# ruanyyyyyyy/point-cloud-process

Hardware: AMD Instinct MI355X
Metric: correspondence-pairs/sec + ms/ICP-iter, 120k-pt KITTI pair (higher is better)
Workload: dtype f64; 1 GPU; point-to-point ICP iteration, 120000 x 120000 KITTI-shaped synthetic scan pair per GPU (BASELINE configs[1]); exact 1-NN via grid; nn=grid, pairs_per_gpu=1, points_src=120000, points_tgt=120000

## Files before the change

include/pcr.h:

```cpp
#ifndef PCR_H
#define PCR_H

#include <stdint.h>

#ifdef __cplusplus
extern "C" {
#endif

#define PCR_API __attribute__((visibility("default")))

enum {
    PCR_OK = 0,
    PCR_E_TOO_FEW_ASSOC = 1,
    PCR_E_INVALID = -1,
    PCR_E_EMPTY = -2,
    PCR_E_NOMEM = -3,
    PCR_E_HIP = -4,
    PCR_E_NO_DEVICE = -5,
    PCR_E_UNSUPPORTED = -6,
    PCR_E_TOO_MANY_ITERS = -7,
    PCR_E_SINGULAR = -8
};

typedef struct pcr_ctx pcr_ctx;
// ... 257 lines not shown
    int32_t reserved_i;
    double inertia;
    double shift;
    double device_ms;
    double reserved[4];
} pcr_kmeans_result;
PCR_API void pcr_kmeans_default_params(pcr_kmeans_params* p);
PCR_API int pcr_kmeans_fit(pcr_ctx* ctx, const pcr_cloud* cloud, const pcr_kmeans_params* params, const double* centers0 ,
                           double* centers_out , int64_t* counts_out , int32_t* labels_out, double* inertia_hist_out,
                           double* shift_hist_out, pcr_kmeans_result* result);
PCR_API int pcr_kmeans_step(pcr_ctx* ctx, const pcr_cloud* cloud, int k, int dim, const double* centers, double* centers_out, int64_t* counts_out,
                            double* sums_out, double* inertia_out, double* shift_out);
PCR_API int pcr_kmeans_predict(pcr_ctx* ctx, const pcr_cloud* cloud, int k, int dim, const double* centers, int32_t* labels_out, int64_t* counts_out,
                               double* inertia_out);
PCR_API int pcr_cloud_download_rows(pcr_ctx* ctx, const pcr_cloud* cloud, const int64_t* rows , int64_t m, double* xyz_out );

PCR_API int pcr_timer_start(pcr_ctx* ctx);
PCR_API int pcr_timer_stop_ms(pcr_ctx* ctx, double* ms_out);
PCR_API int pcr_debug_read(pcr_ctx* ctx, uint64_t* out, int64_t n_words);
PCR_API int pcr_profile_enable(pcr_ctx* ctx, int on);
PCR_API int pcr_search_stats(pcr_ctx* ctx, int64_t out[4]);

PCR_API int pcr_icp_pass_log(pcr_ctx* ctx, int max_n, double* tile_us, double* drain_us, int64_t* items, int* n_out, double host_us[6]);

PCR_API int pcr_ctx_set_shared(pcr_ctx* ctx, int shared);
PCR_API int pcr_profile_read(pcr_ctx* ctx, double ms_out[4], int* passes_out);

#ifdef __cplusplus
}
#endif
#endif
```

point-cloud-process_amd/_lib.py:

```python
from __future__ import annotations

import ctypes as C
import os
import sys

import numpy as np

_HERE = os.path.dirname(os.path.abspath(__file__))
LIB_PATH = os.environ.get("PCR_LIB_PATH") or os.path.join(_HERE, "libpcr.so")

PCR_OK = 0
PCR_E_TOO_FEW_ASSOC = 1
PCR_E_INVALID = -1
PCR_E_EMPTY = -2
PCR_E_NOMEM = -3
PCR_E_HIP = -4
PCR_E_NO_DEVICE = -5
PCR_E_UNSUPPORTED = -6
PCR_E_TOO_MANY_ITERS = -7
PCR_E_SINGULAR = -8

PCR_INDEX_GRID = 0
PCR_INDEX_BRUTE = 1
PCR_ICP_COMPAT_MAIN = 0
# ... 253 lines not shown
    "pcr_prep_download": (C.c_int, [_vp, _vp, _dp, _dp, _dp]),
    "pcr_prep_free": (C.c_int, [_vp, _vp]),
    "pcr_global_registration": (C.c_int, [_vp, _vp, _vp, C.POINTER(RansacParams), C.c_int, C.POINTER(RansacResult)]),
    "pcr_dbscan": (C.c_int, [_vp, _vp, C.c_double, C.c_int, _ip, _ip]),
    "pcr_ground_default_params": (None, [C.POINTER(GroundParams)]),
    "pcr_ground_select": (C.c_int, [_lp, C.c_int32, C.c_int64, C.c_double, _ip, _ip]),
    "pcr_ground_segmentation": (C.c_int, [_vp, _vp, _lp, C.POINTER(GroundParams), C.POINTER(_vp), _ip, C.POINTER(C.c_uint8), _lp, C.POINTER(GroundResult)]),
    "pcr_gmm_default_params": (None, [C.POINTER(GmmParams)]),
    "pcr_gmm_fit": (C.c_int, [_vp, _vp, C.POINTER(GmmParams), _dp, _dp, _dp, _dp, _dp, C.POINTER(GmmResult)]),
    "pcr_gmm_step": (C.c_int, [_vp, _vp, C.c_int, C.c_int, _dp, _dp, _dp, _dp, _dp, _dp, _dp, _dp]),
    "pcr_gmm_predict": (C.c_int, [_vp, _vp, C.c_int, C.c_int, _dp, _dp, _dp, _ip, _dp, _dp]),
    "pcr_gmm_log_density": (C.c_int, [C.c_int, _dp, _dp, _dp, C.c_double, _dp]),
    "pcr_kmeans_default_params": (None, [C.POINTER(KmeansParams)]),
    "pcr_kmeans_fit": (C.c_int, [_vp, _vp, C.POINTER(KmeansParams), _dp, _dp, _lp, _ip, _dp, _dp, C.POINTER(KmeansResult)]),
    "pcr_kmeans_step": (C.c_int, [_vp, _vp, C.c_int, C.c_int, _dp, _dp, _lp, _dp, _dp, _dp]),
    "pcr_kmeans_predict": (C.c_int, [_vp, _vp, C.c_int, C.c_int, _dp, _ip, _lp, _dp]),
    "pcr_cloud_download_rows": (C.c_int, [_vp, _vp, _lp, C.c_int64, _dp]),
    "pcr_debug_read": (C.c_int, [_vp, C.POINTER(C.c_uint64), C.c_int64]),
    "pcr_profile_enable": (C.c_int, [_vp, C.c_int]),
    "pcr_profile_read": (C.c_int, [_vp, _dp, C.POINTER(C.c_int)]),
    "pcr_search_stats": (C.c_int, [_vp, _lp]),
    "pcr_ctx_set_shared": (C.c_int, [_vp, C.c_int]),
    "pcr_icp_pass_log": (C.c_int, [_vp, C.c_int, _dp, _dp, _lp, C.POINTER(C.c_int), _dp]),
    "pcr_timer_start": (C.c_int, [_vp]),
    "pcr_timer_stop_ms": (C.c_int, [_vp, _dp]),
}

_lib = None


class PcrError(RuntimeError):
    def __init__(self, status, detail=""):
        self.status = status
        msg = f"libpcr status {status}"
        try:
            msg += ": " + lib().pcr_strerror(status).decode()
        except Exception:
            pass
        if detail:
            msg += f" ({detail})"
        super().__init__(msg)


def lib():
    global _lib
    if _lib is not None:
# ... 47 lines not shown
```

point-cloud-process_amd/csrc/pcr_core.hip:

```cpp
#include <cmath>
#include <cstdio>
#include <cstring>
#include <cstdlib>
#include <chrono>
#include <thread>
#include <atomic>
#include <memory>
#include "pcr_internal.h"

extern "C" {

const char* pcr_version(void) { return "pcr 0.1 (gfx950, f64)"; }

const char* pcr_strerror(int s) {
    switch (s) {
        case PCR_OK: return "ok";
        case PCR_E_TOO_FEW_ASSOC: return "ICP failed, cannot find enough associations!";
        case PCR_E_INVALID: return "invalid argument";
        case PCR_E_EMPTY: return "empty point cloud";
        case PCR_E_NOMEM: return "out of memory";
        case PCR_E_HIP: return "HIP runtime error";
        case PCR_E_NO_DEVICE: return "no HIP device (libpcr.so needs an AMD GPU; there is no CPU fallback)";
        case PCR_E_UNSUPPORTED: return "unsupported";
        case PCR_E_TOO_MANY_ITERS: return "max_iter exceeds PCR_ICP_MAX_LOG";
// ... 248 lines not shown
    if (!c || !out) return PCR_E_INVALID;
    hipSetDevice(c->device);
    unsigned int fb = 0;
    int rc = pcr_brute_last_fallback(c, &fb);
    if (rc) return rc;
    out[0] = fb;
    out[1] = c->arena_grow_count;
    out[2] = (int64_t)c->arena_grow_us;
    out[3] = (int64_t)c->arenas.size();
    return PCR_OK;
}

int pcr_icp_pass_log(pcr_ctx* c, int max_n, double* tile_us, double* drain_us, int64_t* items, int* n_out, double host_us[6]) {
    if (!c || !n_out || max_n < 0) return PCR_E_INVALID;
    const int n = c->pass_log_n < max_n ? c->pass_log_n : max_n;
    for (int k = 0; k < n; ++k) {
        if (tile_us) tile_us[k] = c->pass_log[0][k];
        if (drain_us) drain_us[k] = c->pass_log[1][k];
        if (items) items[k] = (int64_t)c->pass_log[2][k];
    }
    *n_out = c->pass_log_n;
    if (host_us)
        for (int k = 0; k < 6; ++k) host_us[k] = c->pass_host_us[k];
    return PCR_OK;
}

int pcr_timer_start(pcr_ctx* c) {
    if (!c) return PCR_E_INVALID;
    PCR_HIP(c, hipEventRecord(c->ev2, c->stream));
    return PCR_OK;
}

int pcr_timer_stop_ms(pcr_ctx* c, double* ms) {
    if (!c || !ms) return PCR_E_INVALID;
    PCR_HIP(c, hipEventRecord(c->ev3, c->stream));
    PCR_HIP(c, pcr_event_sync(c->ev3));
    float f = 0;
    PCR_HIP(c, hipEventElapsedTime(&f, c->ev2, c->ev3));
    *ms = f;
    return PCR_OK;
}

}

void pcr_prof_mark(pcr_ctx* ctx, int k) {
    if (ctx->profile) hipEventRecord(ctx->pev[k], ctx->stream);
// ... 324 lines not shown
```

point-cloud-process_amd/csrc/pcr_grid_search.hip:

```cpp
#include <atomic>
#include <chrono>
#include <cmath>
#include <cstdlib>
#include <cstring>
#include "pcr_descent.h"
#include "pcr_icp_step.h"

constexpr unsigned int HARD_SCAN_T = 192;
constexpr int HARD_STACK = 160;
constexpr long long ID_NONE = 0x7fffffffffffffffll;
constexpr int H_NLIST = 32;
constexpr int H_CSTRIDE = 32;
__host__ __device__ static inline unsigned int hard_list_cap(long long nq) {
    const long long halves = (nq + 15) / 16;
    return (unsigned int)(((halves + H_NLIST - 1) / H_NLIST) * 16 + 64);
}

template <int G>
__device__ static inline void group_best(double& bd2, long long& bid, unsigned int& bpos) {
#pragma unroll
    for (int off = G / 2; off > 0; off >>= 1) {
        const double od2 = __shfl_xor(bd2, off, 64);
        const long long oid = __shfl_xor(bid, off, 64);
        const unsigned int opos = __shfl_xor(bpos, off, 64);
// ... 461 lines not shown
    S.won = won;
    S.open = open; S.clamped = clamped; S.qvalid = qvalid;
    S.staged = staged;
    S.dbg_pairs = dbg_pairs; S.dbg_passes = dbg_passes;
    {
        const bool ok = lane < (int)probe_groups && (unsigned int)probe_v == probe_total / (probe_groups ? probe_groups : 1u) + ((unsigned int)lane < probe_total % (probe_groups ? probe_groups : 1u) ? 1u : 0u);
        S.probe = (probe_groups && __ballot(ok) == (probe_groups >= 64 ? ~0ull : (1ull << probe_groups) - 1ull)) ? 1ull : 0ull;
    }
#ifdef PCR_WT_DIAG
    if (dbg) {
        const bool unres = open && lane < WT_Q;
        for (int r = 0; r < 5; ++r) {
            const unsigned int n_r = (unsigned int)__popcll(__ballot(unres && (clamped ? 0 : why) == r));
            if (lane == 0 && n_r) atomicAdd(&dbg[(1 << 15) + r], (unsigned long long)n_r);
        }
        if (lane == 0) {
            t_ph[7] = staged;
            for (int i = 0; i < 8; ++i) dbg[(1 << 16) + (blockIdx.x * 4 + (threadIdx.x >> 6)) * 8 + i] = t_ph[i];
        }
    }
#endif
}

__device__ static inline unsigned int wtile_block(int xcd_remap) {
    unsigned int blk = blockIdx.x;
    if (xcd_remap) {
        const unsigned int per = gridDim.x >> 3, main = per << 3;
        if (blk < main) blk = (blk & 7u) * per + (blk >> 3);
    }
    return blk;
}

__global__ void __launch_bounds__(256) __attribute__((amdgpu_waves_per_eu(PCR_WT_WAVES, 8)))
grid_wtile_kernel(const pcr_grid_view* __restrict__ gvp, pcr_pt* __restrict__ q, long long nq, pcr_xform x, int has_x, int write_back, double max_d2,
                  int gated, int xcd_remap, unsigned int pcap, unsigned int* __restrict__ res_pos, double* __restrict__ res_d2,
                  work_item* __restrict__ hard_list, unsigned int* __restrict__ hard_count, unsigned long long* __restrict__ dbg,
                  const pcr_icp_dev_state* __restrict__ st, const wt_xyz* __restrict__ prev_xyz) {
    __shared__ wtile_lds s_lds[4];
    if (st) {
        if (st->stop) return;
        x = st->x;
    }
    const unsigned long long t_start = dbg ? __builtin_amdgcn_s_memtime() : 0;
    const int lane = threadIdx.x & 63, wave = threadIdx.x >> 6;
    const unsigned int blk = wtile_block(xcd_remap);
    wt_state S;
    wt_pre P;
    wtile_preload(blk * 4 + wave, lane, q, nq, res_pos, prev_xyz, P);
    wtile_search(*gvp, &s_lds[wave], blk * 4 + wave, lane, P, q, nq, x, has_x, write_back, max_d2, gated, pcap, res_pos, res_d2, dbg, prev_xyz, S);
    const bool unres = S.open && lane < WT_Q;
// ... 276 lines not shown
constexpr unsigned long long ITEM_NONE = ~0ull;
constexpr unsigned int POISON_HI = 0xfffffffeu;
__device__ static inline unsigned long long item_poison(unsigned int pass_id) { return ((unsigned long long)POISON_HI << 32) | pass_id; }
#ifndef PCR_PASS_SPIN_LIMIT
#define PCR_PASS_SPIN_LIMIT (1u << 21)
#endif
constexpr unsigned int PASS_SPIN_LIMIT = PCR_PASS_SPIN_LIMIT;
constexpr int Q_BITS = 22;
constexpr unsigned long long Q_MASK = (1ull << Q_BITS) - 1ull;
constexpr long long PASS_MAX_NQ = 1ll << 26;
struct pass_args {
    unsigned long long* items;
    unsigned long long* sync;
    unsigned int cap;
    unsigned long long* acc;
    wt_xyz* prev_xyz;
    double scale, inv_scale;
    pcr_icp_dev_state* st;
    pcr_icp_loop_args la;
    unsigned int* tile_cost;
    unsigned int pass_id;
    unsigned long long* host_block;
    unsigned int notify;
    unsigned int* plog;
};
constexpr int PASS_LOG_WORDS = 3 * PCR_ICP_MAX_LOG + 8;
constexpr size_t HOST_LOG_OFF = (sizeof(pcr_icp_dev_state) + 63) & ~(size_t)63;
constexpr size_t HOST_FLAG_OFF = 8192 - 8;
static_assert(HOST_LOG_OFF + 4 * PASS_LOG_WORDS <= HOST_FLAG_OFF, "state + pass log + flag fit the landing block");
__host__ __device__ static inline unsigned int pass_item_cap(long long nq) {
    const long long tiles = (nq + WT_Q - 1) / WT_Q + 4;
    return (unsigned int)(((tiles + PASS_GROUPS - 1) / PASS_GROUPS) * (WT_Q + 1));
}

__device__ static inline long long to_fixed(double v, double scale) {
    constexpr double BIG = 6755399441055744.0;
    return __double_as_longlong(__builtin_fma(v, scale, BIG)) - __double_as_longlong(BIG);
}

__device__ static inline void acc_fixed_add(unsigned long long* __restrict__ acc, unsigned int set, int lane, double mk, double scale) {
    if (lane < PCR_NMOM - 1 && mk != 0.0)
        atomicAdd(acc + (size_t)(set % ACC_SETS) * PCR_NMOM + lane, (unsigned long long)to_fixed(mk, scale));
}

__device__ static inline void acc_fixed_add_ll(unsigned long long* __restrict__ acc, unsigned int set, int lane, long long v) {
    if (lane < PCR_NMOM - 1 && v != 0) atomicAdd(acc + (size_t)(set % ACC_SETS) * PCR_NMOM + lane, (unsigned long long)v);
}

__device__ static inline unsigned long long ld_dev(const unsigned long long* p) {
    return __hip_atomic_load(p, __ATOMIC_RELAXED, __HIP_MEMORY_SCOPE_AGENT);
}
__device__ static inline void st_dev(unsigned long long* p, unsigned long long v) {
    __hip_atomic_store(p, v, __ATOMIC_RELAXED, __HIP_MEMORY_SCOPE_AGENT);
}

union pass_lds {
    wtile_lds t;
    hard_lds h;
    double xch[WT_Q * (PCR_NMOM - 1)];
    long long xll[WT_Q * (PCR_NMOM - 1)];
};

__device__ __forceinline__ static void pass_serve_item(const pcr_grid_view& gv, pass_lds* L, const int lane, const unsigned long long w, const double max_d2,
                                                       const pass_args& A, unsigned int* __restrict__ res_pos, unsigned long long* __restrict__ dbg,
                                                       const unsigned int dbg_slot, const unsigned long long t_start) {
    const unsigned int w_lo = (unsigned int)w, w_hi = (unsigned int)(w >> 32);
    const double ax = __hiloint2double(__builtin_amdgcn_readlane((int)w_hi, 0), __builtin_amdgcn_readlane((int)w_lo, 0));
    const double ay = __hiloint2double(__builtin_amdgcn_readlane((int)w_hi, 1), __builtin_amdgcn_readlane((int)w_lo, 1));
    const double az = __hiloint2double(__builtin_amdgcn_readlane((int)w_hi, 2), __builtin_amdgcn_readlane((int)w_lo, 2));
    const unsigned int qi = (unsigned int)__builtin_amdgcn_readlane((int)w_lo, 3);
    const float cand_b2 = __uint_as_float((unsigned int)__builtin_amdgcn_readlane((int)w_hi, 3));
    const unsigned long long h_t0 = dbg ? __builtin_amdgcn_s_memtime() : 0;
    unsigned int h_steps = 0, h_pts = 0;
    int s_level0 = 0;
    double bd2;
    long long bid;
    unsigned int bpos;
    const bool have_cand = cand_b2 < INFINITY;
    double win[3];
    hard_search(gv, &L->h, lane, ax, ay, az, have_cand ? fmin((double)cand_b2, max_d2) : max_d2, have_cand, bd2, bid, bpos, h_steps, h_pts, s_level0, win);
    wave_sync();
    if (bpos != POS_NONE) {
        if (lane == 0) {
// ... 155 lines not shown

struct drain_part {
    unsigned int cnt, exc, total;
};
__device__ __forceinline__ static drain_part drain_partition(const unsigned long long* sync, int lane) {
    static_assert(PASS_GROUPS <= 64, "one group per lane");
    drain_part d;
    d.cnt = lane < PASS_GROUPS ? (unsigned int)(sync[(size_t)PASS_SYNC_STRIDE * lane] & Q_MASK) : 0u;
    d.exc = wave_excl_scan_u32(d.cnt, lane, &d.total);
    return d;
}
__device__ __forceinline__ static unsigned long long drain_take(const drain_part& d, unsigned long long* items, unsigned int cap, unsigned int w_i, int lane) {
    const int grp = (int)__ffsll((long long)__ballot(((lane < PASS_GROUPS) & (d.exc <= w_i)) && w_i < d.exc + d.cnt)) - 1;
    const unsigned int idx = w_i - (unsigned int)__builtin_amdgcn_readlane((int)d.exc, grp);
    unsigned long long* it = items + ((size_t)grp * cap + idx) * 4;
    unsigned long long w = ITEM_NONE;
    if (lane < 4) {
        w = it[lane];
        it[lane] = ITEM_NONE;
    }
    return w;
}

#ifndef PCR_PASS_DIAG
#define PCR_PASS_DIAG 0
#endif
__global__ void __launch_bounds__(256) __attribute__((amdgpu_waves_per_eu(PCR_WT_WAVES, 8)))
grid_pass_kernel(const pcr_grid_view* __restrict__ gvp, pcr_grid_view gv, pcr_pt* __restrict__ q, long long nq, double max_d2, int xcd_remap,
                 unsigned int pcap_arg, unsigned int pcap_busy, unsigned int* __restrict__ res_pos, unsigned long long* __restrict__ dbg_arg, int use_prev, int inline_queue,
                 pass_args A) {
    unsigned long long* const dbg = PCR_PASS_DIAG ? dbg_arg : nullptr;
    __shared__ pass_lds s_lds[4];
    const int lane = threadIdx.x & 63, wave = __builtin_amdgcn_readfirstlane((int)(threadIdx.x >> 6));
    const unsigned int tile = wtile_block(xcd_remap) * 4 + wave;
    wt_pre P;
    wtile_preload(tile, lane, q, nq, res_pos, use_prev ? A.prev_xyz : nullptr, P);
    const unsigned int last_cost = use_prev ? A.tile_cost[tile] : 0u;
    unsigned int pcap = pcap_arg;
    if (pcap_busy > pcap_arg && A.plog) {
        const unsigned int prev_items = A.pass_id > 0 && A.pass_id <= (unsigned int)PCR_ICP_MAX_LOG ? A.plog[2 * PCR_ICP_MAX_LOG + A.pass_id - 1] : 0xffffffffu;
        if ((unsigned long long)prev_items * 16ull > (unsigned long long)nq) pcap = pcap_busy;
        pcap = (unsigned int)__builtin_amdgcn_readfirstlane((int)pcap);
    }
    const pcr_xform x = A.st->x;
    if (A.st->stop) return;
    tile_set_priority(last_cost);
    const unsigned long long t_start = dbg ? __builtin_amdgcn_s_memtime() : 0;
    const unsigned long long rt_start = dbg ? __builtin_amdgcn_s_memrealtime() : 0;
    unsigned long long rt_tile = 0, rt_acc = 0;
    unsigned int n_items = 0, n_polls = 0, n_casfail = 0;
    pass_lds* L = &s_lds[wave];
    const unsigned int n_waves = gridDim.x * 4;
    const unsigned int g = tile % PASS_GROUPS;
    const unsigned int g_tiles = n_waves / PASS_GROUPS + (g < n_waves % PASS_GROUPS ? 1u : 0u);
    unsigned long long* const g_q = A.sync + (size_t)PASS_SYNC_STRIDE * g;
    unsigned long long* const g_started = g_q + 16;
    unsigned long long* const g_ticket = g_q + 17;
    unsigned long long* const items = A.items + (size_t)g * A.cap * 4;
    if (lane == 0) __hip_atomic_fetch_add(g_started, 1ull, __ATOMIC_RELAXED, __HIP_MEMORY_SCOPE_AGENT);
    const unsigned int n_groups = n_waves < (unsigned int)PASS_GROUPS ? n_waves : (unsigned int)PASS_GROUPS;
    wt_state S;
    wtile_search(*gvp, &L->t, tile, lane, P, q, nq, x, 1, 1, max_d2, 1, pcap, res_pos, nullptr, dbg, use_prev ? A.prev_xyz : nullptr, S, inline_queue ? A.sync + 16 : nullptr,
                 (unsigned int)PASS_SYNC_STRIDE, n_groups, n_waves);
    tile_record_cost(S, lane, A.tile_cost, tile);
    if (dbg) rt_tile = __builtin_amdgcn_s_memrealtime();
    tile_nb nb;
    tile_neighbour(gv.pts, S, P, lane, nb);
    bool all_started = false;
    if (inline_queue) {
        all_started = S.probe != 0;
        if (!all_started) {
            unsigned long long sv = 0;
            if (lane < (int)n_groups) sv = ld_dev(A.sync + (size_t)PASS_SYNC_STRIDE * lane + 16);
            const bool ok = lane < (int)n_groups && (unsigned int)sv == n_waves / PASS_GROUPS + ((unsigned int)lane < n_waves % PASS_GROUPS ? 1u : 0u);
            all_started = __ballot(ok) == (n_groups >= 64 ? ~0ull : (1ull << n_groups) - 1ull);
// ... 100 lines not shown
        pass_serve_item(gv, L, lane, w, max_d2, A, res_pos, dbg, g + PASS_GROUPS * mine, t_start);
    }
    const unsigned long long rt_loop = dbg ? __builtin_amdgcn_s_memrealtime() : 0;
    asm volatile("s_waitcnt vmcnt(0)" ::: "memory");
    int last = 0;
    {
        if (lane == 0) {
            const unsigned long long tg_old = __hip_atomic_fetch_add(g_ticket, 1ull | (left_by_poison ? 1ull << 32 : 0ull) | (failed ? 1ull << 48 : 0ull), __ATOMIC_RELAXED,
                                                                     __HIP_MEMORY_SCOPE_AGENT);
            if ((unsigned int)tg_old == g_tiles - 1u) {
                const bool g_clean = ((tg_old >> 32) & 0xffffull) != 0 || left_by_poison;
                const bool g_failed = (tg_old >> 48) != 0 || failed;
                const unsigned long long tr_old = __hip_atomic_fetch_add(root, 1ull | (g_clean ? 1ull << 32 : 0ull) | (g_failed ? 1ull << 48 : 0ull), __ATOMIC_RELAXED,
                                                                         __HIP_MEMORY_SCOPE_AGENT);
                if ((unsigned int)tr_old == n_groups - 1u) {
                    last = ((unsigned int)((tr_old >> 32) & 0xffffull) + (g_clean ? 1u : 0u) == n_groups) ? 1 : 2;
                    if ((tr_old >> 48) != 0 || g_failed) last = 3;
                }
            }
        }
    }
    if (dbg && lane == 0) {
        unsigned long long* d = dbg + (1 << 19) + (size_t)(blockIdx.x * 4 + wave) * 8;
        d[0] = rt_start; d[1] = rt_tile; d[2] = rt_acc; d[3] = rt_loop; d[4] = n_items; d[5] = n_polls | ((unsigned long long)n_casfail << 32); d[6] = S.dbg_pairs | ((unsigned long long)S.dbg_passes << 40) | ((unsigned long long)__popcll(um) << 48); d[7] = __builtin_amdgcn_s_memrealtime();
    }
    last = __builtin_amdgcn_readfirstlane(last);
    if (!last) return;
    if (last == 3 && dbg_arg && lane == 0) atomicAdd(&dbg_arg[(1 << 19) - 16], 1ull);
    if (last >= 2) {
        unsigned long long qw = 0;
        if (lane < (int)n_groups) qw = ld_dev(A.sync + (size_t)PASS_SYNC_STRIDE * lane);
        const unsigned int r_l = (unsigned int)(qw & Q_MASK);
        const unsigned int c_l = last == 3 ? 0u : (unsigned int)((qw >> Q_BITS) & Q_MASK);
        unsigned long long left = __ballot(lane < (int)n_groups && c_l < r_l);
        while (left) {
            const int gg = (int)__ffsll((long long)left) - 1;
            left &= left - 1;
            const unsigned int c0 = (unsigned int)__builtin_amdgcn_readlane((int)c_l, gg), r0 = (unsigned int)__builtin_amdgcn_readlane((int)r_l, gg);
            for (unsigned int i = c0; i < r0; ++i) {
                unsigned long long* it = A.items + ((size_t)gg * A.cap + i) * 4;
                unsigned long long w = ITEM_NONE;
                bool arrived = false;
                const unsigned int patience = last == 3 ? 64u : (PASS_SPIN_LIMIT < (1u << 21) ? (1u << 21) : PASS_SPIN_LIMIT);
                bool served_before = false;
                for (unsigned int spins = 0; spins < patience; ++spins) {
                    if (lane < 4) w = ld_dev(it + lane);
                    const unsigned int w3_hi = (unsigned int)__builtin_amdgcn_readlane((int)(unsigned int)(w >> 32), 3);
// ... 188 lines not shown
        __syncthreads();
        if (threadIdx.x == 0) pcr::icp_step(st, s_m, gv.origin, la, st->r_diff, st->t_diff);
    }
}

struct grid_scratch {
    pcr_dev_block res_pos, res_d2;
    pcr_dev_block hard_list;
    pcr_dev_block prev_xyz;
    pcr_dev_block acc, items, tile_cost;
    unsigned int* const hard_count;
    explicit grid_scratch(pcr_ctx* ctx)
        : res_pos(ctx), res_d2(ctx), hard_list(ctx), prev_xyz(ctx), acc(ctx), items(ctx), tile_cost(ctx), hard_count(ctx->d_counters + PCR_HARD_COUNTERS) {}
};

static int grid_scratch_alloc(grid_scratch* sc, int64_t nq, bool want_d2, bool want_hard) {
    int rc;
    if ((rc = sc->res_pos.alloc(sizeof(unsigned int) * nq))) return rc;
    if (want_d2 && (rc = sc->res_d2.alloc(sizeof(double) * nq))) return rc;
    if (want_hard && (rc = sc->hard_list.alloc(sizeof(work_item) * (size_t)H_NLIST * hard_list_cap(nq)))) return rc;
    return PCR_OK;
}

struct pass_layout {
    size_t sync_word, log_word, zero_words;
    unsigned int cap;
    unsigned long long item_words;
};
static pass_layout pass_scratch_layout(long long nq, int n_pairs, bool with_log) {
    pass_layout l;
    l.sync_word = (size_t)n_pairs * ACC_SETS * PCR_NMOM;
    l.log_word = l.sync_word + PASS_SYNC_WORDS;
    l.zero_words = l.log_word + (with_log ? PASS_LOG_WORDS / 2 : 0);
    l.cap = pass_item_cap(nq);
    l.item_words = 4ull * PASS_GROUPS * l.cap;
    return l;
}

static int wtile_blocks(int64_t nq) { return (int)((nq + 4 * WT_Q - 1) / (4 * WT_Q)); }
static int queue_blocks(const pcr_ctx* ctx, long long want) { return (int)(want < 8ll * ctx->cu_count ? (want < 1 ? 1 : want) : 8ll * ctx->cu_count); }

static unsigned int wtile_point_cap(const pcr_ctx* ctx, int64_t nq) {
    const int nblocks = (int)((nq + 63) / 64);
    return (unsigned int)WT_PR * (nblocks > 8 * ctx->cu_count ? WT_ROUNDS_LARGE : WT_ROUNDS_SMALL);
}
constexpr unsigned int WT_BUSY_CAP = WT_PR * 48;
constexpr int WT_XCD_REMAP = 1;

static int grid_search_enqueue(pcr_ctx* ctx, const pcr_index* idx, pcr_pt* q, int64_t nq, hipStream_t stream, const pcr_xform* x, int write_back,
                               double max_d2, bool gated, bool mark, const grid_scratch* sc, const pcr_icp_dev_state* st, bool use_prev = false) {
    const int nblocks = (int)((nq + 63) / 64);
    pcr_xform xi;
    pcr_xform_from_T(nullptr, &xi);
    if (mark) pcr_prof_mark(ctx, 0);
    {
        if (ctx->d_debug) hipMemsetAsync(ctx->d_debug, 0, sizeof(unsigned long long) * ((1 << 16) + 8 * (size_t)nblocks), stream);
        hipLaunchKernelGGL(grid_wtile_kernel, dim3(wtile_blocks(nq)), dim3(256), 0, stream, (const pcr_grid_view*)idx->d_view, q, (long long)nq, x ? *x : xi,
                           (x || st) ? 1 : 0, write_back, max_d2, gated ? 1 : 0, WT_XCD_REMAP, wtile_point_cap(ctx, nq), sc->res_pos.as<unsigned int>(),
                           sc->res_d2.as<double>(), sc->hard_list.as<work_item>(), sc->hard_count, ctx->d_debug, st, (const wt_xyz*)(use_prev ? sc->prev_xyz.p : nullptr));
    }
    if (mark) pcr_prof_mark(ctx, 1);
    hipLaunchKernelGGL(grid_hard_kernel, dim3(queue_blocks(ctx, (nq + 3) / 4)), dim3(256), 0, stream, idx->view, (const work_item*)sc->hard_list.p,
// ... 77 lines not shown
    frexp(M / (double)nq, &exq);
    const int F = (61 - ex < 51 - exq) ? 61 - ex : 51 - exq;
    if (!(M > 0) || !std::isfinite(M) || F < 20) return false;
    *scale = ldexp(1.0, F);
    *inv_scale = ldexp(1.0, -F);
    return true;
}

static std::atomic<int> g_loops_in_flight[64];
struct loop_guard {
    std::atomic<int>& n;
    explicit loop_guard(int device) : n(g_loops_in_flight[(unsigned int)device % 64u]) { n.fetch_add(1); }
    ~loop_guard() { n.fetch_sub(1); }
};

int pcr_grid_icp_loop(pcr_ctx* ctx, const pcr_index* idx, pcr_cloud* qc, const pcr_icp_params* params, const double T0[16],
                      pcr_icp_result* res) {
    const loop_guard in_flight(ctx->device);
    const auto h_t0 = std::chrono::steady_clock::now();
    auto h_us = [&](std::chrono::steady_clock::time_point a) { return std::chrono::duration_cast<std::chrono::nanoseconds>(std::chrono::steady_clock::now() - a).count() / 1e3; };
    for (double& v : ctx->pass_host_us) v = 0.0;
    const char* const wait_s = getenv("PCR_PASS_INLINE");
    const int wait_env = wait_s ? atoi(wait_s) : -1;
    const bool gated = (params->max_d2 > 0) && std::isfinite(params->max_d2);
    int rc = pcr_cloud_morton_sort(ctx, qc, idx->cell);
    if (rc) return rc;
    const int64_t nq = qc->n;
    int grid = (int)((nq + 1023) / 1024);
    if (grid > ctx->cu_count) grid = ctx->cu_count;
    double sc_f = 0, sc_i = 0;
    const bool fused = gated && nq <= PASS_MAX_NQ && getenv("PCR_ICP_NO_FUSED") == nullptr &&
                       pcr_pass_fixed_scale(idx->lo, idx->hi, nq, params->max_d2, &sc_f, &sc_i);
    grid_scratch sc(ctx);
    pcr_dev_block st_blk(ctx);
    if ((rc = grid_scratch_alloc(&sc, nq, false, !fused)) || (rc = sc.prev_xyz.alloc(24 * (size_t)nq))) return rc;
    const pass_layout pl = pass_scratch_layout(nq, 1, true);
    pass_args pa{};
    if (fused) {
        if ((rc = sc.acc.alloc(8 * pl.zero_words)) || (rc = sc.tile_cost.alloc(sizeof(unsigned int) * 4 * (size_t)wtile_blocks(nq))) ||
            (rc = sc.items.alloc(8 * pl.item_words)))
            return rc;
        pa.cap = pl.cap;
        pa.items = sc.items.as<unsigned long long>();
        pa.tile_cost = sc.tile_cost.as<unsigned int>();
        pa.acc = sc.acc.as<unsigned long long>();
        pa.sync = pa.acc + pl.sync_word;
        pa.plog = (unsigned int*)(pa.acc + pl.log_word);
        pa.prev_xyz = sc.prev_xyz.as<wt_xyz>();
        pa.scale = sc_f;
        pa.inv_scale = sc_i;
    }
    if ((rc = pcr_ensure_scratch(ctx, sizeof(double) * PCR_NMOM * (size_t)grid)) || (rc = st_blk.alloc(sizeof(pcr_icp_dev_state)))) return rc;
    pcr_icp_dev_state* const d_st = st_blk.as<pcr_icp_dev_state>();
    static_assert(sizeof(pcr_icp_dev_state) <= 8192, "state must fit the pinned staging buffer");
    pcr_icp_dev_state* h_st = (pcr_icp_dev_state*)ctx->h_state;
    memset(h_st, 0, sizeof(*h_st));
    pcr::icp_state_from_T0(T0, h_st);
    const pcr_icp_loop_args la = pcr_icp_loop_args_from(params);
    volatile unsigned long long* const h_flag = (volatile unsigned long long*)((char*)ctx->h_state + HOST_FLAG_OFF);
    if (fused) {
        void* dp = nullptr;
        if (hipHostGetDevicePointer(&dp, ctx->h_state, 0) == hipSuccess) pa.host_block = (unsigned long long*)dp;
        *h_flag = 0ull;
        h_flag[-1] = 0ull;
    }
    hipError_t e = hipSuccess;
    ctx->pass_host_us[0] = h_us(h_t0);
    if (fused) {
        pass_T0 t0;
        for (int i = 0; i < 16; ++i) t0.v[i] = T0[i];
        const int ib = (int)((pl.item_words + 256 * 8 - 1) / (256 * 8));
        hipLaunchKernelGGL(pass_init_kernel, dim3(ib < 1 ? 1 : (ib > 1024 ? 1024 : ib)), dim3(256), 0, ctx->stream, pa.acc, (unsigned int)pl.zero_words,
                           pa.items, pl.item_words, d_st, t0, pa.plog,
                           pa.host_block ? pa.host_block + HOST_FLAG_OFF / 8 - 1 : (unsigned long long*)nullptr);
        e = hipGetLastError();
    } else e = hipMemcpyAsync(d_st, h_st, sizeof(*h_st), hipMemcpyHostToDevice, ctx->stream);
    pa.st = d_st;
    pa.la = la;
    pcr_xform xi;
    pcr_xform_from_T(nullptr, &xi);
    int enq = 0;
    const double prof_before = ctx->prof_ms[0] + ctx->prof_ms[1] + ctx->prof_ms[2] + ctx->prof_ms[3];
    int chunk = params->min_iter > 2 ? params->min_iter : 2;
    if (ctx->profile) chunk = 1;
    while (e == hipSuccess && rc == PCR_OK && enq < params->max_iter) {
        if (chunk > params->max_iter - enq) chunk = params->max_iter - enq;
        if (chunk > 64) chunk = 64;
        for (int c = 0; c < chunk && rc == PCR_OK; ++c) {
            const bool use_prev = enq + c > 0;
            const bool one_generation = (nq + WT_Q - 1) / WT_Q <= 16ll * ctx->cu_count;
            const int inline_queue = wait_env >= 0 ? wait_env : ((one_generation && !ctx->shared_device && in_flight.n.load(std::memory_order_relaxed) == 1) ? 1 : 0);
            if (fused) {
                if (ctx->profile) pcr_prof_mark(ctx, 0);
                if (ctx->d_debug) hipMemsetAsync(ctx->d_debug, 0, sizeof(unsigned long long) * (inline_queue ? ((1 << 16) + 8 * (size_t)((nq + 63) / 64)) : ((size_t)1 << 19)), ctx->stream);
                pa.pass_id = (unsigned int)(enq + c);
                pa.notify = c == chunk - 1 ? 1u : 0u;
                const unsigned int cap_n = wtile_point_cap(ctx, nq), cap_busy = (!inline_queue && cap_n > (unsigned int)(WT_PR * WT_ROUNDS_SMALL)) ? WT_BUSY_CAP : cap_n;
                hipLaunchKernelGGL(grid_pass_kernel, dim3(wtile_blocks(nq)), dim3(256), 0, ctx->stream, (const pcr_grid_view*)idx->d_view, idx->view, qc->d, (long long)nq,
                                   params->max_d2, WT_XCD_REMAP, cap_n, cap_busy, sc.res_pos.as<unsigned int>(), ctx->d_debug, use_prev ? 1 : 0, inline_queue, pa);
                if (ctx->profile) pcr_prof_mark(ctx, 1);
                if (!inline_queue)
                    hipLaunchKernelGGL(grid_drain_kernel, dim3(queue_blocks(ctx, (nq + 3) / 4)), dim3(256), 0, ctx->stream, idx->view, params->max_d2,
                                       sc.res_pos.as<unsigned int>(), ctx->d_debug, pa);
                if (hipGetLastError() != hipSuccess) { rc = PCR_E_HIP; break; }
                pcr_prof_mark(ctx, 2);
            } else {
                rc = grid_search_enqueue(ctx, idx, qc->d, nq, ctx->stream, nullptr, 1, params->max_d2, gated, ctx->profile, &sc, d_st, use_prev);
                if (rc) break;
                pcr_prof_mark(ctx, 2);
                hipLaunchKernelGGL(grid_accumulate_kernel, dim3(grid), dim3(256), 0, ctx->stream, idx->view, (const pcr_pt*)qc->d, (long long)nq, xi,
                                   0, (const unsigned int*)sc.res_pos.p, params->max_d2, gated ? 1 : 0, ctx->d_partials, ctx->d_counters + 64,
                                   (double*)nullptr, sc.hard_count, d_st, la, sc.prev_xyz.as<wt_xyz>());
            }
            pcr_prof_mark(ctx, 3);
            pcr_prof_mark(ctx, 4);
            pcr_prof_finish(ctx);
        }
        enq += chunk;
        if (rc) break;
        if (ctx->pass_host_us[1] == 0.0) ctx->pass_host_us[1] = h_us(h_t0) - ctx->pass_host_us[0];
        const auto h_tw = std::chrono::steady_clock::now();
// ... 7 lines not shown
                __builtin_ia32_pause();
            }
            ctx->pass_host_us[5] = h_us(h_tw);
            if (!seen) {
                e = pcr_sync(ctx->stream);
                if (e == hipSuccess && pcr_d2h_small(ctx, h_st, d_st, sizeof(*h_st)) != PCR_OK) e = hipErrorUnknown;
            }
        } else {
            hipEventRecord(ctx->ev3, ctx->stream);
            if (pcr_d2h_small_enqueue(ctx, h_st, d_st, sizeof(*h_st)) != PCR_OK) e = hipErrorUnknown;
            if (e == hipSuccess && fused && pcr_d2h_small_enqueue(ctx, (char*)ctx->h_state + HOST_LOG_OFF, pa.plog, 4 * PASS_LOG_WORDS) != PCR_OK) e = hipErrorUnknown;
            double flag_us = 0.0;
            if (e == hipSuccess && pcr_wait_flag(ctx, &flag_us) != PCR_OK) e = hipErrorUnknown;
            ctx->pass_host_us[5] = flag_us;
            { float ms = 0; if (hipEventElapsedTime(&ms, ctx->ev0, ctx->ev3) == hipSuccess) ctx->pass_host_us[4] = 1e3 * ms; }
        }
        ctx->pass_host_us[2] += h_us(h_tw);
        if (e != hipSuccess || h_st->stop) break;
        if (!ctx->profile) chunk *= 2;
    }
    if (e == hipSuccess) e = hipGetLastError();
    ctx->pass_log_n = 0;
    ctx->loop_dev_ms = 0.0;
    if (e == hipSuccess && rc == PCR_OK && fused) {
        const unsigned int* const lg = (const unsigned int*)((const char*)ctx->h_state + HOST_LOG_OFF);
        const int np = h_st->passes < PCR_ICP_MAX_LOG ? h_st->passes : PCR_ICP_MAX_LOG;
        unsigned int prev = lg[3 * PCR_ICP_MAX_LOG];
        for (int k = 0; k < np; ++k) {
            const unsigned int end = lg[k], ds = lg[PCR_ICP_MAX_LOG + k];
            ctx->pass_log[0][k] = 0.01 * (double)(unsigned int)((ds ? ds : end) - prev);
            ctx->pass_log[1][k] = ds ? 0.01 * (double)(unsigned int)(end - ds) : 0.0;
            ctx->pass_log[2][k] = (double)lg[2 * PCR_ICP_MAX_LOG + k];
            prev = end;
        }
        ctx->pass_log_n = np;
        ctx->loop_dev_ms = np > 0 ? 1e-5 * (double)(unsigned int)(lg[np - 1] - lg[3 * PCR_ICP_MAX_LOG]) : 0.0;
    }
    ctx->pass_host_us[3] = h_us(h_t0);
    if (rc) return rc;
    if (e != hipSuccess) { ctx->last_error = hipGetErrorString(e); return PCR_E_HIP; }
    if (h_st->status == PCR_E_HIP) { ctx->last_error = "ICP pass: a wave gave up waiting on the work queue"; return PCR_E_HIP; }
    if ((rc = pcr_icp_finish(ctx, qc, params, h_st, res))) return rc;
    res->nn_kernel_ms = ctx->profile ? (ctx->prof_ms[0] + ctx->prof_ms[1] + ctx->prof_ms[2] + ctx->prof_ms[3]) - prof_before : 0.0;
    return PCR_OK;
}

__device__ static inline const pcr_batch_pair* batch_pair_ptr(const pcr_batch_pass_args& B, unsigned int p) {
    return as_global(B.pairs) + p;
}

__global__ void __launch_bounds__(256) __attribute__((amdgpu_waves_per_eu(PCR_WT_WAVES, 8)))
batch_pass_kernel(pcr_batch_pass_args B, int xcd_remap, unsigned int pcap, unsigned int pass_id, int use_prev) {
    __shared__ pass_lds s_lds[4];
    const int lane = threadIdx.x & 63, wave = __builtin_amdgcn_readfirstlane((int)(threadIdx.x >> 6));
    const unsigned int tile_g = (unsigned int)__builtin_amdgcn_readfirstlane((int)(wtile_block(xcd_remap) * 4 + wave));
    const unsigned int p = (unsigned int)__builtin_amdgcn_readfirstlane((int)as_global(B.tile_pair)[tile_g]);
    if (p >= (unsigned int)B.n_pairs) return;
    const pcr_batch_pair* const bp = batch_pair_ptr(B, p);
// ... 122 lines not shown
```

point-cloud-process_amd/csrc/pcr_internal.h:

```cpp
#pragma once
#include <hip/hip_runtime.h>
#include <stdint.h>
#include <string>
#include <vector>
#include "pcr.h"

#define PCR_HIDDEN __attribute__((visibility("hidden")))

struct __attribute__((aligned(32))) pcr_pt {
    double x, y, z;
    long long id;
};

struct pcr_xform {
    double r[9];
    double t[3];
};

constexpr int PCR_MAX_LEVELS = 12;
constexpr int PCR_COORD_BITS = 21;
constexpr long long PCR_COORD_BIAS = 1ll << 20;
constexpr long long PCR_COORD_MAX = (1ll << PCR_COORD_BITS) - 1;
constexpr unsigned long long PCR_EMPTY_KEY = ~0ull;

// ... 72 lines not shown
    void* h_state = nullptr;
    void* h_small = nullptr;
    void* h_big = nullptr;
    size_t h_big_bytes = 0;
    void* h_stage = nullptr;
    size_t h_stage_bytes = 0;
    void* h_init = nullptr;
    size_t h_init_bytes = 0;
    void* h_down = nullptr;
    size_t h_down_half = 0;
    size_t h_pinned_bytes = 0;
    int shared_device = 0;
    double* d_partials = nullptr;
    size_t d_partials_bytes = 0;
    unsigned int* d_counters = nullptr;
    unsigned int* d_cell_counts = nullptr;
    unsigned long long* d_debug = nullptr;
    bool profile = false;
    hipEvent_t pev[5] = {nullptr, nullptr, nullptr, nullptr, nullptr};
    double prof_ms[4] = {0, 0, 0, 0};
    int prof_passes = 0;
    double pass_log[3][PCR_ICP_MAX_LOG];
    int pass_log_n = 0;
    double loop_dev_ms = 0.0;
    double pass_host_us[6] = {0, 0, 0, 0, 0, 0};
    int cu_count = 256;
    char name[256] = {0};
    int64_t hbm_bytes = 0;
};

#include <chrono>
static inline hipError_t pcr_sync(hipStream_t s) {
    const auto t0 = std::chrono::steady_clock::now();
    for (unsigned int spins = 0;; ++spins) {
        const hipError_t e = hipStreamQuery(s);
        if (e != hipErrorNotReady) return e;
        if ((spins & 1023u) == 1023u && std::chrono::steady_clock::now() - t0 > std::chrono::seconds(2)) return hipStreamSynchronize(s);
        __builtin_ia32_pause();
    }
}
static inline hipError_t pcr_event_sync(hipEvent_t ev) {
    const auto t0 = std::chrono::steady_clock::now();
    for (unsigned int spins = 0;; ++spins) {
        const hipError_t e = hipEventQuery(ev);
        if (e != hipErrorNotReady) return e;
        if ((spins & 1023u) == 1023u && std::chrono::steady_clock::now() - t0 > std::chrono::seconds(2)) return hipEventSynchronize(ev);
// ... 124 lines not shown
```

point-cloud-process_amd/device.py:

```python
from __future__ import annotations

import ctypes as C
import threading

import numpy as np

from . import _lib as L

_default_ctx = {}
_lock = threading.Lock()


class Context:

    def __init__(self, device=0, shared=False):
        self._h = C.c_void_p()
        self.device = int(device)
        L.check(L.lib().pcr_ctx_create(self.device, C.byref(self._h)))
        if shared:
            self.set_shared(True)

    def set_shared(self, shared=True):
        L.check(L.lib().pcr_ctx_set_shared(self.handle, 1 if shared else 0), self.handle)

# ... 17 lines not shown
        L.check(L.lib().pcr_timer_start(self.handle), self.handle)

    def timer_stop_ms(self):
        ms = C.c_double()
        L.check(L.lib().pcr_timer_stop_ms(self.handle, C.byref(ms)), self.handle)
        return ms.value

    def profile(self, on=True):
        L.check(L.lib().pcr_profile_enable(self.handle, 1 if on else 0), self.handle)

    def profile_read(self):
        ms = np.zeros(4)
        n = C.c_int()
        L.check(L.lib().pcr_profile_read(self.handle, L.dptr(ms), C.byref(n)), self.handle)
        return ms, n.value

    def pass_log(self):
        t, d, it, n = np.zeros(L.PCR_ICP_MAX_LOG), np.zeros(L.PCR_ICP_MAX_LOG), np.zeros(L.PCR_ICP_MAX_LOG, dtype=np.int64), C.c_int()
        h = np.zeros(6)
        L.check(L.lib().pcr_icp_pass_log(self.handle, L.PCR_ICP_MAX_LOG, L.dptr(t), L.dptr(d), L.lptr(it), C.byref(n), L.dptr(h)), self.handle)
        k = min(n.value, L.PCR_ICP_MAX_LOG)
        return {"tile_us": t[:k].tolist(), "drain_us": d[:k].tolist(), "items": it[:k].tolist(),
                "host_us": {"setup": h[0], "enqueue_first_chunk": h[1], "waiting_for_device": h[2], "whole_loop": h[3], "events_start_to_last_kernel": h[4], "last_wait": h[5]}}

    def search_stats(self):
        out = np.zeros(4, dtype=np.int64)
        L.check(L.lib().pcr_search_stats(self.handle, L.lptr(out)), self.handle)
        return {"brute_fallback": int(out[0]), "arena_allocations": int(out[1]), "arena_allocation_us": int(out[2]), "arenas": int(out[3])}

    def close(self):
        if self._h:
            L.lib().pcr_ctx_destroy(self._h)
            self._h = C.c_void_p()

    def __del__(self):
        try:
            self.close()
        except Exception:
            pass


def default_context(device=0):
    with _lock:
        ctx = _default_ctx.get(device)
        if ctx is None:
            ctx = Context(device)
# ... 264 lines not shown
```

Before: 3.359 billion correspondences/s.

## Deal tile blocks across CUs by previous-pass cost via on-device sorted permutation

Adds 8 extra blocks to the grid pass kernel that, using per-tile costs from the previous ICP pass, bitonic-sort each XCD's tile blocks by cost and greedily assign them to CUs to balance load. The next pass reads the double-buffered permutation to remap block indices. The aim is to cut tail imbalance from uneven NN search work across CUs. It adds a small sort and extra launch blocks per pass, and relies on the assumption that blocks are dispatched round-robin to CUs in a predictable way.

Result: slower. 3.273 billion correspondences/s (-2.6%).

```diff
diff --git a/include/pcr.h b/include/pcr.h
--- a/include/pcr.h
+++ b/include/pcr.h
@@ -303,6 +303,7 @@
 PCR_API int pcr_search_stats(pcr_ctx* ctx, int64_t out[4]);
 
 PCR_API int pcr_icp_pass_log(pcr_ctx* ctx, int max_n, double* tile_us, double* drain_us, int64_t* items, int* n_out, double host_us[6]);
+PCR_API int pcr_icp_deal_log(pcr_ctx* ctx, int64_t* passes, int64_t* moved);
 
 PCR_API int pcr_ctx_set_shared(pcr_ctx* ctx, int shared);
 PCR_API int pcr_profile_read(pcr_ctx* ctx, double ms_out[4], int* passes_out);
diff --git a/point-cloud-process_amd/_lib.py b/point-cloud-process_amd/_lib.py
--- a/point-cloud-process_amd/_lib.py
+++ b/point-cloud-process_amd/_lib.py
@@ -299,6 +299,7 @@
     "pcr_search_stats": (C.c_int, [_vp, _lp]),
     "pcr_ctx_set_shared": (C.c_int, [_vp, C.c_int]),
     "pcr_icp_pass_log": (C.c_int, [_vp, C.c_int, _dp, _dp, _lp, C.POINTER(C.c_int), _dp]),
+    "pcr_icp_deal_log": (C.c_int, [_vp, C.POINTER(C.c_int64), C.POINTER(C.c_int64)]),
     "pcr_timer_start": (C.c_int, [_vp]),
     "pcr_timer_stop_ms": (C.c_int, [_vp, _dp]),
 }
diff --git a/point-cloud-process_amd/csrc/pcr_core.hip b/point-cloud-process_amd/csrc/pcr_core.hip
--- a/point-cloud-process_amd/csrc/pcr_core.hip
+++ b/point-cloud-process_amd/csrc/pcr_core.hip
@@ -294,6 +294,13 @@
     *n_out = c->pass_log_n;
     if (host_us)
         for (int k = 0; k < 6; ++k) host_us[k] = c->pass_host_us[k];
+    return PCR_OK;
+}
+
+int pcr_icp_deal_log(pcr_ctx* c, int64_t* passes, int64_t* moved) {
+    if (!c || !passes || !moved) return PCR_E_INVALID;
+    *passes = (int64_t)c->deal_log[0];
+    *moved = (int64_t)c->deal_log[1];
     return PCR_OK;
 }
 
diff --git a/point-cloud-process_amd/csrc/pcr_grid_search.hip b/point-cloud-process_amd/csrc/pcr_grid_search.hip
--- a/point-cloud-process_amd/csrc/pcr_grid_search.hip
+++ b/point-cloud-process_amd/csrc/pcr_grid_search.hip
@@ -507,10 +507,10 @@
 #endif
 }
 
-__device__ static inline unsigned int wtile_block(int xcd_remap) {
+__device__ static inline unsigned int wtile_block(int xcd_remap, unsigned int n_blk = gridDim.x) {
     unsigned int blk = blockIdx.x;
     if (xcd_remap) {
-        const unsigned int per = gridDim.x >> 3, main = per << 3;
+        const unsigned int per = n_blk >> 3, main = per << 3;
         if (blk < main) blk = (blk & 7u) * per + (blk >> 3);
     }
     return blk;
@@ -833,6 +833,9 @@
     unsigned int pass_id;
     unsigned long long* host_block;
     unsigned int notify;
+    const unsigned int* perm_rd;
+    unsigned int* perm_wr;
+    unsigned int n_tile_blocks, deal_cus;
     unsigned int* plog;
 };
 constexpr int PASS_LOG_WORDS = 3 * PCR_ICP_MAX_LOG + 8;
@@ -870,6 +873,7 @@
     hard_lds h;
     double xch[WT_Q * (PCR_NMOM - 1)];
     long long xll[WT_Q * (PCR_NMOM - 1)];
+    unsigned int deal[128];
 };
 
 __device__ __forceinline__ static void pass_serve_item(const pcr_grid_view& gv, pass_lds* L, const int lane, const unsigned long long w, const double max_d2,
@@ -1071,6 +1075,68 @@
     return w;
 }
 
+
+constexpr unsigned int DEAL_MAX = 128;
+constexpr unsigned int DEAL_TILE_BASE = 512;
+constexpr unsigned int DEAL_OPEN_WEIGHT = 8;
+static_assert(4 * (DEAL_TILE_BASE + 0xffffu + DEAL_OPEN_WEIGHT * WT_Q) < (1u << 19), "block cost | index fits a 32-bit sort key, unit sum | lane a positive int");
+__device__ __noinline__ static unsigned int deal_build(unsigned int* __restrict__ keys, const unsigned int* __restrict__ tile_cost, unsigned int* __restrict__ perm,
+                                               const unsigned int n_blk, const unsigned int run, const unsigned int n_cus, const int lane) {
+    const unsigned int per = n_blk >> 3, main = per << 3, base = run * per;
+    if (run == 0 && (unsigned int)lane < n_blk - main) perm[main + lane] = main + lane;
+    bool ok = n_cus >= 1u && n_cus <= 64u && per >= n_cus && per <= DEAL_MAX;
+    unsigned int key[2] = {0u, 0u};
+    bool bad = false;
+    if (ok) {
+#pragma unroll
+        for (int u = 0; u < 2; ++u) {
+            const unsigned int i = (unsigned int)lane + 64u * u;
+            if (i < per) {
+                unsigned int cost = 0;
+#pragma unroll
+                for (int t = 0; t < 4; ++t) {
+                    const unsigned int w = tile_cost[(size_t)(base + i) * 4 + t];
+                    bad = bad || (w >> 16) > (unsigned int)WT_Q;
+                    cost += DEAL_TILE_BASE + (w & 0xffffu) + DEAL_OPEN_WEIGHT * (w >> 16);
+                }
+                key[u] = (cost << 7) | (127u - i);
+            }
+        }
+    }
+    if (!ok || __any(bad)) {
+        for (unsigned int i = lane; i < per; i += 64) perm[base + i] = base + i;
+        return 0u;
+    }
+    keys[lane] = key[0];
+    keys[lane + 64] = key[1];
+    wave_sync();
+#pragma unroll 1
+    for (unsigned int k = 2; k <= 128; k <<= 1) {
+#pragma unroll 1
+        for (unsigned int j = k >> 1; j > 0; j >>= 1) {
+            const unsigned int t = (((unsigned int)lane & ~(j - 1u)) << 1) | ((unsigned int)lane & (j - 1u)), p = t | j;
+            const unsigned int a = keys[t], b = keys[p];
+            if ((a < b) == ((t & k) == 0u)) { keys[t] = b; keys[p] = a; }
+            wave_sync();
+        }
+    }
+    const unsigned int places = (unsigned int)lane < n_cus ? (per - (unsigned int)lane + n_cus - 1u) / n_cus : 0u;
+    unsigned int sum = 0, used = 0, moved = 0;
+#pragma unroll 1
+    for (unsigned int r = 0; r < per; ++r) {
+        const unsigned int kk = keys[r];
+        const int c = wave_min_i32(used < places ? (int)((sum << 6) | (unsigned int)lane) : 0x7fffffff) & 63;
+        if (lane == c) {
+            const unsigned int at = (unsigned int)lane + n_cus * used, b = 127u - (kk & 127u);
+            perm[base + at] = base + b;
+            moved += at != b ? 1u : 0u;
+            sum += kk >> 7;
+            ++used;
+        }
+    }
+    return moved;
+}
+
 #ifndef PCR_PASS_DIAG
 #define PCR_PASS_DIAG 0
 #endif
@@ -1081,7 +1147,20 @@
     unsigned long long* const dbg = PCR_PASS_DIAG ? dbg_arg : nullptr;
     __shared__ pass_lds s_lds[4];
     const int lane = threadIdx.x & 63, wave = __builtin_amdgcn_readfirstlane((int)(threadIdx.x >> 6));
-    const unsigned int tile = wtile_block(xcd_remap) * 4 + wave;
+    const unsigned int n_blk = A.n_tile_blocks;
+    if (blockIdx.x >= n_blk) {
+        if (wave == 0 && A.perm_wr && !A.st->stop) {
+            const unsigned int moved = deal_build(s_lds[0].deal, A.tile_cost, A.perm_wr, n_blk, blockIdx.x - n_blk, A.deal_cus, lane);
+            if (A.plog && moved) __hip_atomic_fetch_add(A.plog + 3 * PCR_ICP_MAX_LOG + 1, moved, __ATOMIC_RELAXED, __HIP_MEMORY_SCOPE_AGENT);
+        }
+        return;
+    }
+    unsigned int blk = wtile_block(xcd_remap, n_blk);
+    if (A.perm_rd) {
+        const unsigned int pb = *(const __attribute__((address_space(4))) unsigned int*)(unsigned long long)(A.perm_rd + blk);
+        blk = pb < n_blk ? pb : blk;
+    }
+    const unsigned int tile = blk * 4 + wave;
     wt_pre P;
     wtile_preload(tile, lane, q, nq, res_pos, use_prev ? A.prev_xyz : nullptr, P);
     const unsigned int last_cost = use_prev ? A.tile_cost[tile] : 0u;
@@ -1097,9 +1176,10 @@
     const unsigned long long t_start = dbg ? __builtin_amdgcn_s_memtime() : 0;
     const unsigned long long rt_start = dbg ? __builtin_amdgcn_s_memrealtime() : 0;
     unsigned long long rt_tile = 0, rt_acc = 0;
+    const unsigned int hw_id = dbg ? __builtin_amdgcn_s_getreg(4 | (31 << 11)) : 0u, hw_xcc = dbg ? __builtin_amdgcn_s_getreg(20 | (3 << 11)) : 0u;
     unsigned int n_items = 0, n_polls = 0, n_casfail = 0;
     pass_lds* L = &s_lds[wave];
-    const unsigned int n_waves = gridDim.x * 4;
+    const unsigned int n_waves = n_blk * 4;
     const unsigned int g = tile % PASS_GROUPS;
     const unsigned int g_tiles = n_waves / PASS_GROUPS + (g < n_waves % PASS_GROUPS ? 1u : 0u);
     unsigned long long* const g_q = A.sync + (size_t)PASS_SYNC_STRIDE * g;
@@ -1246,7 +1326,7 @@
     }
     if (dbg && lane == 0) {
         unsigned long long* d = dbg + (1 << 19) + (size_t)(blockIdx.x * 4 + wave) * 8;
-        d[0] = rt_start; d[1] = rt_tile; d[2] = rt_acc; d[3] = rt_loop; d[4] = n_items; d[5] = n_polls | ((unsigned long long)n_casfail << 32); d[6] = S.dbg_pairs | ((unsigned long long)S.dbg_passes << 40) | ((unsigned long long)__popcll(um) << 48); d[7] = __builtin_amdgcn_s_memrealtime();
+        d[0] = rt_start; d[1] = rt_tile; d[2] = rt_acc; d[3] = rt_loop; d[4] = (unsigned long long)n_items | ((unsigned long long)(hw_id & 0xffffu) << 16) | ((unsigned long long)(hw_xcc & 0xfu) << 32) | ((unsigned long long)tile << 36); d[5] = n_polls | ((unsigned long long)n_casfail << 32); d[6] = S.dbg_pairs | ((unsigned long long)S.dbg_passes << 40) | ((unsigned long long)__popcll(um) << 48); d[7] = __builtin_amdgcn_s_memrealtime();
     }
     last = __builtin_amdgcn_readfirstlane(last);
     if (!last) return;
@@ -1481,8 +1561,9 @@
     return PCR_OK;
 }
 
+static int wtile_blocks(int64_t nq) { return (int)((nq + 4 * WT_Q - 1) / (4 * WT_Q)); }
 struct pass_layout {
-    size_t sync_word, log_word, zero_words;
+    size_t sync_word, log_word, perm_word, zero_words;
     unsigned int cap;
     unsigned long long item_words;
 };
@@ -1490,13 +1571,13 @@
     pass_layout l;
     l.sync_word = (size_t)n_pairs * ACC_SETS * PCR_NMOM;
     l.log_word = l.sync_word + PASS_SYNC_WORDS;
-    l.zero_words = l.log_word + (with_log ? PASS_LOG_WORDS / 2 : 0);
+    l.perm_word = l.log_word + (with_log ? (PASS_LOG_WORDS + 1) / 2 : 0);
+    l.zero_words = l.perm_word + (with_log ? (size_t)wtile_blocks(nq) : 0);
     l.cap = pass_item_cap(nq);
     l.item_words = 4ull * PASS_GROUPS * l.cap;
     return l;
 }
 
-static int wtile_blocks(int64_t nq) { return (int)((nq + 4 * WT_Q - 1) / (4 * WT_Q)); }
 static int queue_blocks(const pcr_ctx* ctx, long long want) { return (int)(want < 8ll * ctx->cu_count ? (want < 1 ? 1 : want) : 8ll * ctx->cu_count); }
 
 static unsigned int wtile_point_cap(const pcr_ctx* ctx, int64_t nq) {
@@ -1620,6 +1701,8 @@
     for (double& v : ctx->pass_host_us) v = 0.0;
     const char* const wait_s = getenv("PCR_PASS_INLINE");
     const int wait_env = wait_s ? atoi(wait_s) : -1;
+    const char* const deal_s = getenv("PCR_TILE_DEAL");
+    const bool deal_env = !(deal_s && atoi(deal_s) == 0);
     const bool gated = (params->max_d2 > 0) && std::isfinite(params->max_d2);
     int rc = pcr_cloud_morton_sort(ctx, qc, idx->cell);
     if (rc) return rc;
@@ -1644,6 +1727,8 @@
         pa.acc = sc.acc.as<unsigned long long>();
         pa.sync = pa.acc + pl.sync_word;
         pa.plog = (unsigned int*)(pa.acc + pl.log_word);
+        pa.n_tile_blocks = (unsigned int)wtile_blocks(nq);
+        pa.deal_cus = (unsigned int)(ctx->cu_count / 8);
         pa.prev_xyz = sc.prev_xyz.as<wt_xyz>();
         pa.scale = sc_f;
         pa.inv_scale = sc_i;
@@ -1678,6 +1763,8 @@
     pcr_xform xi;
     pcr_xform_from_T(nullptr, &xi);
     int enq = 0;
+    bool deal_built = false;
+    long long dealt_passes = 0;
     const double prof_before = ctx->prof_ms[0] + ctx->prof_ms[1] + ctx->prof_ms[2] + ctx->prof_ms[3];
     int chunk = params->min_iter > 2 ? params->min_iter : 2;
     if (ctx->profile) chunk = 1;
@@ -1693,8 +1780,15 @@
                 if (ctx->d_debug) hipMemsetAsync(ctx->d_debug, 0, sizeof(unsigned long long) * (inline_queue ? ((1 << 16) + 8 * (size_t)((nq + 63) / 64)) : ((size_t)1 << 19)), ctx->stream);
                 pa.pass_id = (unsigned int)(enq + c);
                 pa.notify = c == chunk - 1 ? 1u : 0u;
+                const int n_tb = wtile_blocks(nq);
+                const bool deal = deal_env && inline_queue && use_prev && pa.deal_cus >= 1u && pa.deal_cus <= 64u && 4ll * (n_tb + 8) <= 16ll * ctx->cu_count;
+                unsigned int* const perm = (unsigned int*)(pa.acc + pl.perm_word);
+                pa.perm_rd = deal && deal_built ? perm + (size_t)(pa.pass_id & 1u) * n_tb : nullptr;
+                pa.perm_wr = deal ? perm + (size_t)((pa.pass_id + 1u) & 1u) * n_tb : nullptr;
+                deal_built = deal;
+                if (pa.perm_rd) ++dealt_passes;
                 const unsigned int cap_n = wtile_point_cap(ctx, nq), cap_busy = (!inline_queue && cap_n > (unsigned int)(WT_PR * WT_ROUNDS_SMALL)) ? WT_BUSY_CAP : cap_n;
-                hipLaunchKernelGGL(grid_pass_kernel, dim3(wtile_blocks(nq)), dim3(256), 0, ctx->stream, (const pcr_grid_view*)idx->d_view, idx->view, qc->d, (long long)nq,
+                hipLaunchKernelGGL(grid_pass_kernel, dim3(n_tb + (deal ? 8 : 0)), dim3(256), 0, ctx->stream, (const pcr_grid_view*)idx->d_view, idx->view, qc->d, (long long)nq,
                                    params->max_d2, WT_XCD_REMAP, cap_n, cap_busy, sc.res_pos.as<unsigned int>(), ctx->d_debug, use_prev ? 1 : 0, inline_queue, pa);
                 if (ctx->profile) pcr_prof_mark(ctx, 1);
                 if (!inline_queue)
@@ -1748,6 +1842,7 @@
     if (e == hipSuccess) e = hipGetLastError();
     ctx->pass_log_n = 0;
     ctx->loop_dev_ms = 0.0;
+    ctx->deal_log[0] = ctx->deal_log[1] = 0;
     if (e == hipSuccess && rc == PCR_OK && fused) {
         const unsigned int* const lg = (const unsigned int*)((const char*)ctx->h_state + HOST_LOG_OFF);
         const int np = h_st->passes < PCR_ICP_MAX_LOG ? h_st->passes : PCR_ICP_MAX_LOG;
@@ -1760,6 +1855,8 @@
             prev = end;
         }
         ctx->pass_log_n = np;
+        ctx->deal_log[0] = dealt_passes;
+        ctx->deal_log[1] = (long long)lg[3 * PCR_ICP_MAX_LOG + 1];
         ctx->loop_dev_ms = np > 0 ? 1e-5 * (double)(unsigned int)(lg[np - 1] - lg[3 * PCR_ICP_MAX_LOG]) : 0.0;
     }
     ctx->pass_host_us[3] = h_us(h_t0);
diff --git a/point-cloud-process_amd/csrc/pcr_internal.h b/point-cloud-process_amd/csrc/pcr_internal.h
--- a/point-cloud-process_amd/csrc/pcr_internal.h
+++ b/point-cloud-process_amd/csrc/pcr_internal.h
@@ -118,6 +118,7 @@
     int prof_passes = 0;
     double pass_log[3][PCR_ICP_MAX_LOG];
     int pass_log_n = 0;
+    long long deal_log[2] = {0, 0};
     double loop_dev_ms = 0.0;
     double pass_host_us[6] = {0, 0, 0, 0, 0, 0};
     int cu_count = 256;
diff --git a/point-cloud-process_amd/device.py b/point-cloud-process_amd/device.py
--- a/point-cloud-process_amd/device.py
+++ b/point-cloud-process_amd/device.py
@@ -63,6 +63,11 @@
         k = min(n.value, L.PCR_ICP_MAX_LOG)
         return {"tile_us": t[:k].tolist(), "drain_us": d[:k].tolist(), "items": it[:k].tolist(),
                 "host_us": {"setup": h[0], "enqueue_first_chunk": h[1], "waiting_for_device": h[2], "whole_loop": h[3], "events_start_to_last_kernel": h[4], "last_wait": h[5]}}
+
+    def deal_log(self):
+        p, m = C.c_int64(), C.c_int64()
+        L.check(L.lib().pcr_icp_deal_log(self.handle, C.byref(p), C.byref(m)), self.handle)
+        return {"passes": int(p.value), "moved": int(m.value)}
 
     def search_stats(self):
         out = np.zeros(4, dtype=np.int64)
```
